# danihae/bio-image-unet

Hardware: AMD Instinct MI355X
Metric: voxels/sec fwd+bwd (higher is better)
Workload: dtype bf16; 1 GPU; cfg4: UNet3D(in_channels=1, out_channels=1, n_filter=32) input (4, 1, 128, 128, 128) per GPU, train step = forward + reference loss + backward + Adam; parallelism=dp1

## Files before the change

### bio_image_unet_amd/csrc/biu_api.hip

```cpp
#include "biu_common.h"
#include "biu_internal.h"

#include <stdlib.h>
#include <string.h>

static const char* const kOffTokens[] = {
    "conv_fwd", "conv_dgrad", "conv_wgrad", "convt_fwd", "convt_dgrad", "convt_wgrad", "convt_all", "c1", "c1_mfma", "cat",
    "fused_stats", "wgrad_bn", "dgrad_bnred", "pool_pair", "pool_pipe", "pool_bnred", "head_bnred", "ksplit", "m16", "m16x2", "rr16",
    "wroll", "wroll16", "wroll2d", "upconv", "foldt", "foldall", "foldck8", "foldgemm", "croll", "froll", "prepack", "wsplitbn",
    "capturefork", "sidechain",
};
constexpr int kNumOffTokens = sizeof(kOffTokens) / sizeof(kOffTokens[0]);
static_assert(kNumOffTokens <= 64, "BiuEnv::off holds one bit per token");

static int off_index(const char* tok, size_t n) {
    for (int i = 0; i < kNumOffTokens; ++i)
        if (strlen(kOffTokens[i]) == n && strncmp(kOffTokens[i], tok, n) == 0) return i;
    return -1;
}
static void env_unknown(const char* var, const char* val, int n) {
    fprintf(stderr, "[biu] %s: unknown %s '%.*s' ignored\n", var, strcmp(var, "BIU_DISABLE") == 0 ? "token" : "value", n, val);
}
static bool parse_int(const char* s, int* v) {
    char* end = nullptr;
    const long r = strtol(s, &end, 10);
    if (end == s || *end) return false;
    *v = (int)r;
    return true;
}

const BiuEnv& biu_env() {
    static const BiuEnv env = [] {
        BiuEnv v{0, false, false, 0, 2, 0, 128};
        if (const char* p = getenv("BIU_DISABLE")) {
            while (true) {
                const size_t n = strcspn(p, ",");
                const int i = off_index(p, n);
                if (i >= 0) v.off |= 1ull << i;
                else if (n > 0) env_unknown("BIU_DISABLE", p, (int)n);
                if (!p[n]) break;
                p += n + 1;
            }
        }
        if (const char* e = getenv("BIU_ROLL"); e && *e) {
            if (strcmp(e, "always") == 0) v.roll_always = true;
            else env_unknown("BIU_ROLL", e, (int)strlen(e));
        }
        if (const char* e = getenv("BIU_FOLDT"); e && *e) {
            int n = 0;
            if (strcmp(e, "always") == 0) v.foldt_always = true;
            else if (strncmp(e, "cmax:", 5) == 0 && parse_int(e + 5, &n) && n > 0) v.foldt_cmax = n;
            else if (strcmp(e, "size") != 0) env_unknown("BIU_FOLDT", e, (int)strlen(e));
        }
        if (const char* e = getenv("BIU_FP32_PRODUCTS"); e && *e) {
            if (strcmp(e, "exact") == 0) v.fp32_products = 0;
            else if (strcmp(e, "bf16x3") == 0) v.fp32_products = 1;
            else if (strcmp(e, "bf16x6") != 0) env_unknown("BIU_FP32_PRODUCTS", e, (int)strlen(e));
        }
        if (const char* e = getenv("BIU_FP32_PRODUCTS_3D"); e && *e) {
            if (strcmp(e, "bf16x3") == 0) v.fp32_products_3d = 1;
            else if (strcmp(e, "bf16x6") == 0) v.fp32_products_3d = 2;
            else if (strcmp(e, "exact") != 0) env_unknown("BIU_FP32_PRODUCTS_3D", e, (int)strlen(e));
// ... 497 lines not shown
```

### bio_image_unet_amd/csrc/biu_conv_mfma.hip

```cpp
#include "biu_internal.h"
#include <type_traits>
#include <cstring>
#include <mutex>
#include <cstdlib>

typedef float floatx16 __attribute__((ext_vector_type(16)));
typedef float floatx4 __attribute__((ext_vector_type(4)));
typedef __bf16 bf16x8 __attribute__((ext_vector_type(8)));

template <typename T> struct Frag;
template <> struct Frag<bf16_t> {
    static constexpr int PE = 8;
    __device__ static __forceinline__ void mma(const uint4& a, const uint4& b, floatx16& c) {
        c = __builtin_amdgcn_mfma_f32_32x32x16_bf16(__builtin_bit_cast(bf16x8, a), __builtin_bit_cast(bf16x8, b), c, 0, 0, 0);
    }
    __device__ static __forceinline__ void unpack(const uint4& v, float* f) {
        const unsigned u[4] = {v.x, v.y, v.z, v.w};
#pragma unroll
        for (int i = 0; i < 4; ++i) {
            f[2 * i] = __uint_as_float(u[i] << 16);
            f[2 * i + 1] = __uint_as_float(u[i] & 0xffff0000u);
        }
    }
    __device__ static __forceinline__ uint4 pack(const float* f) {
// ... 2964 lines not shown
            if (tap < TAPS) {
#pragma unroll
                for (int ni = 0; ni < NI; ++ni)
#pragma unroll
                    for (int e = 0; e < 16; ++e) {
                        const int ii = it * CTA + ni * CT + (e & 3) + 8 * (e >> 2) + 4 * hf;
                        if (ii < a.CA) atomicAdd(wsp + ((size_t)tap * a.CA + ii) * a.CB + jj, acc[t2][ni][e]);
                    }
            }
        }
    }
}

typedef unsigned v4u_t __attribute__((ext_vector_type(4)));
__device__ __forceinline__ void bload_lds16(unsigned voff, v4u_t rsrc, unsigned lds_base_uniform) {
    unsigned keep;
    asm volatile("s_mov_b32 %0, m0\n\ts_mov_b32 m0, %3\n\ts_nop 0\n\tbuffer_load_dwordx4 %1, %2, 0 offen lds\n\ts_mov_b32 m0, %0"
                 : "=&s"(keep)
                 : "v"(voff), "s"(rsrc), "s"(lds_base_uniform)
                 : "memory");
}
__device__ __forceinline__ v4u_t raw_rsrc(const void* base, unsigned bytes) {
    const unsigned long long pa = (unsigned long long)base;
    v4u_t r;
    r[0] = __builtin_amdgcn_readfirstlane((unsigned)pa);
    r[1] = __builtin_amdgcn_readfirstlane((unsigned)(pa >> 32) & 0xffffu);
    r[2] = __builtin_amdgcn_readfirstlane(bytes);
    r[3] = 0x00020000u;
    return r;
}

#ifndef BIU_WROLL_ABL
#define BIU_WROLL_ABL 0
#endif
#ifndef BIU_DIAG_WAVE
#define BIU_DIAG_WAVE 0
#endif
constexpr int WR_TD = 2, WR_TH = 8, WR_TW = 16;
constexpr int WR_HH = WR_TH + 2, WR_HW = WR_TW + 2, WR_PL = WR_HH * WR_HW;
constexpr int WR_RS = 64;
constexpr int WR_PLB = WR_PL * WR_RS;
constexpr int WR_NBI = 24;
constexpr int WR_PAIRB = WR_NBI * 1024;
constexpr int WR_NPAIR = 4;
constexpr int WR_BV = WR_TD * WR_TH * WR_TW;
constexpr int WR_AB = WR_BV * WR_RS;
constexpr int WR_NAI = WR_AB / 1024;
constexpr int WR_NABUF = 3;
constexpr size_t WR_LDS = (size_t)WR_NPAIR * WR_PAIRB + WR_NABUF * WR_AB + 9 * 32 * sizeof(float);

__device__ __forceinline__ unsigned opaque_s(unsigned x) { asm volatile("" : "+s"(x)); return x; }
template <int N> __device__ __forceinline__ void wait_vmcnt() { asm volatile("s_waitcnt vmcnt(%0)" ::"n"(N) : "memory"); }

template <bool BNF, bool K2D, bool A16 = false>
__global__ __launch_bounds__(512, 2) void k_wgrad_roll(WgradArgs a) {
    static_assert(!(K2D && A16), "the 16-channel plain operand form exists for volumes only");
    using T = bf16_t;
    using F = Frag<T>;
    constexpr int TD = WR_TD, TH = WR_TH, TW = WR_TW, HW = WR_HW, PL = WR_PL, RS = WR_RS, PLB = WR_PLB, PAIRB = WR_PAIRB;
    constexpr int CT = 32, PE = 8, TAPS = K2D ? 9 : 27, IPW = K2D ? 3 : 4, NROW = TD * TH;
    constexpr int NBK = WR_NBI / 8, NAK = A16 ? 1 : WR_NAI / 8;
    constexpr int NACC = A16 ? 6 : IPW;

    extern __shared__ __attribute__((aligned(16))) uint4 lds[];
    char* bring = (char*)lds;
    char* abuf = bring + WR_NPAIR * PAIRB;
    float* lxf = (float*)(abuf + WR_NABUF * WR_AB);
    constexpr int LB = 0, LBN = 3 * CT;

    const int tid = threadIdx.x, lane = tid & 63;
    const int wave = __builtin_amdgcn_readfirstlane(tid >> 6);
    const int it = blockIdx.y / a.jt_count, jt = a.jt_begin + blockIdx.y % a.jt_count;
    const int piece = lane & 3;
    const int apc = A16 ? (piece & 1) : piece;
    const int ac0 = it * CT + apc * PE, bc0 = jt * CT + piece * PE;
    const bool apiece_ok = ac0 < a.CA, bpiece_ok = bc0 < a.CB;
    const bool b_src1 = a.pb1 && jt * CT >= a.bsplit;
    const char* pb_ = b_src1 ? a.pb1 : a.pb;
    const int bpitch_ = b_src1 ? a.bpitch1 : a.bpitch;
    const int bc_local = bc0 - (b_src1 ? a.bsplit : 0);
    const float* bs_ = b_src1 ? a.bs1_ : a.bs_;
    const float* bb_ = b_src1 ? a.bb1_ : a.bb_;
    const float* bl_ = b_src1 ? a.bl1_ : a.bl_;
    const bool b_xf = bs_ != nullptr;
    constexpr bool bn_fused = BNF;
    const bool wb = bn_fused && a.write_back;
    if (tid < CT && bn_fused) {
        const int ca = it * CT + tid;
        const bool ok = ca < a.CA;
        lxf[LBN + 0 * CT + tid] = ok ? a.bn_scale[ca] : 1.f;
        lxf[LBN + 1 * CT + tid] = ok ? a.bn_shift[ca] : 0.f;
        lxf[LBN + 2 * CT + tid] = (ok && a.bn_slope) ? a.bn_slope[ca] : 1.f;
        lxf[LBN + 3 * CT + tid] = ok ? a.bn_cA[ca] : 0.f;
        lxf[LBN + 4 * CT + tid] = ok ? a.bn_cB[ca] : 0.f;
        lxf[LBN + 5 * CT + tid] = ok ? a.bn_cC[ca] : 0.f;
    }
    if (tid < CT) {
        const int cb = jt * CT + tid;
        const int cbl = cb - (b_src1 ? a.bsplit : 0);
        lxf[LB + 0 * CT + tid] = (b_xf && cb < a.CB) ? bs_[cbl] : 1.f;
        lxf[LB + 1 * CT + tid] = (b_xf && cb < a.CB) ? bb_[cbl] : 0.f;
        lxf[LB + 2 * CT + tid] = (b_xf && cb < a.CB) ? bl_[cbl] : 1.f;
    }

    floatx16 acc[NACC];
#pragma unroll
    for (int t = 0; t < NACC; ++t)
#pragma unroll
        for (int e = 0; e < 16; ++e) acc[t][e] = 0.f;
    const int wkd = wave / 3, wkw = wave % 3;
    const bool has_x = A16 ? (wave < 4) : (!K2D && wave < 3);
    int tapid[IPW];
#pragma unroll
    for (int t = 0; t < IPW; ++t) {
        if constexpr (K2D) tapid[t] = (wave < 6) ? t * 3 + wkw : TAPS;
        else tapid[t] = (t < 3) ? (wkd * 3 + t) * 3 + wkw : (has_x ? (2 * 3 + wave) * 3 + 2 : TAPS);
    }
    int ab_lane;
    {
        const int g = lane >> 4, li = lane & 15, qrow = li >> 2, p = li & 3, cg = g & 1, h = g >> 1;
        ab_lane = (8 * h + qrow) * RS + (16 * cg + 4 * p) * 2;
    }

    unsigned bco[NBK], aco[NAK];
#pragma unroll
    for (int k = 0; k < NBK; ++k) {
        const int v = ((wave + 8 * k) * 64 + lane) >> 2;
        const int pl = v / PL, r = v % PL;
        bco[k] = (v < 2 * PL && bpiece_ok) ? (unsigned)(pl | ((r / HW) << 10) | ((r % HW) << 20)) : 0xffffffffu;
    }
#pragma unroll
    for (int k = 0; k < NAK; ++k) {
        const int v = ((wave + 8 * k) * 64 + lane) >> 2;
        if constexpr (A16) aco[k] = apiece_ok ? (unsigned)((piece >> 1) | ((v >> 4) << 10) | ((v & 15) << 20)) : 0xffffffffu;
        else aco[k] = apiece_ok ? (unsigned)((v >> 7) | (((v >> 4) & 7) << 10) | ((v & 15) << 20)) : 0xffffffffu;
    }
    const unsigned rowA = (unsigned)a.apitch * 2u, rowY = (unsigned)a.ypitch * 2u, rowB = (unsigned)bpitch_ * 2u;
    const size_t sampA = (size_t)a.GD * a.GH * a.GW * rowA, sampY = (size_t)a.GD * a.GH * a.GW * rowY, sampB = (size_t)a.BD * a.BH * a.BW * rowB;
    const unsigned lds0 = (unsigned)(uintptr_t)((__attribute__((address_space(3))) void*)bring);

    int cn = 0, ch0 = 0, cw0 = 0;
    v4u_t rsB, rsA;
    __amdgpu_buffer_rsrc_t rsAr, rsYr;
    struct Slot { unsigned bmask, amask; uint4 pa[BNF ? NAK : 1], pyv[BNF ? NAK : 1]; };
    Slot sl0, sl1;
    sl0.bmask = sl0.amask = sl1.bmask = sl1.amask = 0;
    unsigned bbase[NBK], abase_[NAK], ybase_[BNF ? NAK : 1];
    unsigned planeB = 0, planeA = 0, planeY = 0;
    auto set_column = [&](int col) __attribute__((always_inline)) {
        int c = col;
        const int wb_ = c % a.nbw; c /= a.nbw;
        const int hb = c % a.nbh;
        cn = c / a.nbh;
        ch0 = hb * TH; cw0 = wb_ * TW;
        rsB = raw_rsrc(pb_ + (size_t)cn * sampB, (unsigned)sampB);
        rsA = raw_rsrc(a.pa + (size_t)cn * sampA, (unsigned)sampA);
        rsAr = __builtin_amdgcn_make_buffer_rsrc((void*)(a.pa + (size_t)cn * sampA), 0, (int)(unsigned)sampA, 0x00020000);
        rsYr = __builtin_amdgcn_make_buffer_rsrc((void*)(a.py + (size_t)cn * sampY), 0, bn_fused ? (int)(unsigned)sampY : 0, 0x00020000);
        planeB = (unsigned)(a.BH * a.BW) * rowB; planeA = (unsigned)(a.GH * a.GW) * rowA; planeY = (unsigned)(a.GH * a.GW) * rowY;
#pragma unroll
        for (int k = 0; k < NBK; ++k) {
            const unsigned x = bco[k];
            const int gh = ch0 - 1 + (int)((x >> 10) & 1023u), gw = cw0 - 1 + (int)(x >> 20);
            const bool ok = x != 0xffffffffu && (unsigned)gh < (unsigned)a.BH && (unsigned)gw < (unsigned)a.BW;
            bbase[k] = ok ? (unsigned)(gh * a.BW + gw) * rowB + (unsigned)bc_local * 2u + (x & 1023u) * planeB : 0xffffffffu;
        }
#pragma unroll
        for (int k = 0; k < NAK; ++k) {
            const unsigned x = aco[k];
            const int gh = ch0 + (int)((x >> 10) & 1023u), gw = cw0 + (int)(x >> 20);
            const bool ok = x != 0xffffffffu && gh < a.GH && gw < a.GW;
            const unsigned vox = (unsigned)(gh * a.GW + gw);
            abase_[k] = ok ? vox * rowA + (unsigned)ac0 * 2u + (x & 1023u) * planeA : 0xffffffffu;
            if constexpr (BNF) ybase_[k] = ok ? vox * rowY + (unsigned)ac0 * 2u + (x & 1023u) * planeY : 0xffffffffu;
        }
    };
    struct FetchCtx { int pair, buf; bool bd0, bd1, ad0, ad1; unsigned dofB, dofA, dofY; };
    auto fetch_ctx = [&](int pair, int gp0, int buf, int d0) __attribute__((always_inline)) -> FetchCtx {
        FetchCtx f;
        f.pair = pair; f.buf = buf;
        f.bd0 = (unsigned)gp0 < (unsigned)a.BD; f.bd1 = (unsigned)(gp0 + 1) < (unsigned)a.BD;
        f.ad0 = d0 < a.GD; f.ad1 = d0 + 1 < a.GD;
        f.dofB = opaque_s((unsigned)gp0 * planeB);
        f.dofA = opaque_s((unsigned)d0 * planeA); f.dofY = opaque_s((unsigned)d0 * planeY);
        f.pair = (int)opaque_s((unsigned)pair); f.buf = (int)opaque_s((unsigned)buf);
        return f;
    };
    auto fetch_piece = [&](Slot& sl, const FetchCtx& f, int i) __attribute__((always_inline)) {
        if (i < NBK) {
            const int k = i;
            const bool ok = bbase[k] != 0xffffffffu && ((bco[k] & 1u) ? f.bd1 : f.bd0);
            bload_lds16(ok ? bbase[k] + f.dofB : 0xffffffffu, rsB, lds0 + (unsigned)(f.pair * PAIRB + (wave + 8 * k) * 1024));
            sl.bmask = (k == 0 ? 0u : sl.bmask) | (ok ? (1u << k) : 0u);
        } else {
            const int k = i - NBK;
            const bool ok = abase_[k] != 0xffffffffu && ((aco[k] & 1u) ? f.ad1 : f.ad0);
            if constexpr (BNF) {
                const auto v0 = __builtin_amdgcn_raw_buffer_load_b128(rsAr, ok ? (int)(abase_[k] + f.dofA) : -1, 0, 0);
                const auto v1 = __builtin_amdgcn_raw_buffer_load_b128(rsYr, ok ? (int)(ybase_[k] + f.dofY) : -1, 0, 0);
                sl.pa[k] = make_uint4(v0[0], v0[1], v0[2], v0[3]);
                sl.pyv[k] = make_uint4(v1[0], v1[1], v1[2], v1[3]);
            } else {
                bload_lds16(ok ? abase_[k] + f.dofA : 0xffffffffu, rsA, lds0 + (unsigned)(WR_NPAIR * PAIRB + f.buf * WR_AB + (wave + 8 * k) * 1024));
            }
            sl.amask = (k == 0 ? 0u : sl.amask) | (ok ? (1u << k) : 0u);
        }
    };
    auto fetch_all = [&](Slot& sl, const FetchCtx& f, bool with_a) __attribute__((always_inline)) {
#pragma unroll
        for (int i = 0; i < NBK + NAK; ++i)
            if (i < NBK || with_a) fetch_piece(sl, f, i);
    };
    auto finish = [&](Slot& sl, int pair_, int buf_, int d0, bool with_a) __attribute__((always_inline)) {
        const int pair = (int)opaque_s((unsigned)pair_), buf = (int)opaque_s((unsigned)buf_);
        const unsigned dofA = opaque_s((unsigned)d0 * planeA);
        if (b_xf) {
            float sc[PE], sh[PE], sl_[PE];
#pragma unroll
            for (int e = 0; e < PE; ++e) { sc[e] = lxf[LB + piece * PE + e]; sh[e] = lxf[LB + CT + piece * PE + e]; sl_[e] = lxf[LB + 2 * CT + piece * PE + e]; }
#pragma unroll
            for (int k = 0; k < NBK; ++k) {
                if ((sl.bmask >> k) & 1u) {
                    uint4* p_ = (uint4*)(bring + pair * PAIRB + (wave + 8 * k) * 1024 + lane * 16);
                    *p_ = apply_xf16<T, PE>(*p_, sc, sh, sl_);
                }
            }
        }
        __builtin_amdgcn_sched_barrier(0);
        if constexpr (BNF) if (with_a) {
            {
                float ks[PE], kh[PE], kl[PE];
#pragma unroll
                for (int e = 0; e < PE; ++e) { ks[e] = lxf[LBN + apc * PE + e]; kh[e] = lxf[LBN + CT + apc * PE + e]; kl[e] = lxf[LBN + 2 * CT + apc * PE + e]; }
#pragma unroll
                for (int k = 0; k < NAK; ++k) {
                    if ((sl.amask >> k) & 1u) {
                        float g[PE], yy[PE];
                        F::unpack(sl.pa[k], g);
                        F::unpack(sl.pyv[k], yy);
#pragma unroll
                        for (int e = 0; e < PE; ++e) g[e] *= (fmaf(ks[e], yy[e], kh[e]) > 0.f ? 1.f : kl[e]);
                        sl.pa[k] = F::pack(g);
                    }
                }
            }
            __builtin_amdgcn_sched_barrier(0);
            {
                float ka[PE], kb[PE], kc[PE];
#pragma unroll
                for (int e = 0; e < PE; ++e) { ka[e] = lxf[LBN + 3 * CT + apc * PE + e]; kb[e] = lxf[LBN + 4 * CT + apc * PE + e]; kc[e] = lxf[LBN + 5 * CT + apc * PE + e]; }
#pragma unroll
                for (int k = 0; k < NAK; ++k) {
                    uint4 v = make_uint4(0, 0, 0, 0);
                    const bool ok = (sl.amask >> k) & 1u;
                    if (ok) {
                        float g[PE], yy[PE];
                        F::unpack(sl.pa[k], g);
                        F::unpack(sl.pyv[k], yy);
#pragma unroll
                        for (int e = 0; e < PE; ++e) g[e] = fmaf(ka[e], g[e], fmaf(kb[e], yy[e], kc[e]));
                        v = F::pack(g);
                    }
                    if (wb) __builtin_amdgcn_raw_buffer_store_b128(v4u_t{v.x, v.y, v.z, v.w}, rsAr, ok ? (int)(abase_[k] + dofA) : -1, 0, 0);
                    *(uint4*)(abuf + buf * WR_AB + (wave + 8 * k) * 1024 + lane * 16) = v;
                }
            }
        }
    };
    auto wait_older = [&](bool younger_in_flight) __attribute__((always_inline)) {
        if (!younger_in_flight) { wait_vmcnt<0>(); return; }
        if (wb) wait_vmcnt<NAK + NBK + 2 * NAK>();
        else if (bn_fused) wait_vmcnt<NBK + 2 * NAK>();
        else wait_vmcnt<NBK + NAK>();
    };

    typedef bf16x4 __attribute__((address_space(3))) * lp;
    auto rd = [&](const char* p_) -> bf16x8 {
        const bf16x4 v0 = __builtin_amdgcn_ds_read_tr16_b64_v4bf16((lp)(p_));
        const bf16x4 v1 = __builtin_amdgcn_ds_read_tr16_b64_v4bf16((lp)(p_ + 4 * RS));
        return __builtin_shufflevector(v0, v1, 0, 1, 2, 3, 4, 5, 6, 7);
    };
    auto mfma_step = [&](auto has_x_c, int s4, int buf, auto&& issue) __attribute__((always_inline)) {
        constexpr bool HAS_X = decltype(has_x_c)::value;
        auto pj = [&](int j) -> const char* { return bring + opaque_s((unsigned)(((s4 + (j >> 1)) & 3) * PAIRB + (j & 1) * PLB)); };
        if constexpr (A16) {
            const int uj = wave & 3, ukw = wave >> 2;
            const char* b0 = pj(uj) + ukw * RS + ab_lane;
            const char* c0 = pj(uj) + 2 * RS + ab_lane;
            const char* ab = abuf + opaque_s((unsigned)(buf * WR_AB)) + ab_lane;
            bf16x8 ring[4], ring2[HAS_X ? 4 : 1], faa[2];
            faa[0] = rd(ab);
#pragma unroll
            for (int j = 0; j < 3; ++j) {
                ring[j] = rd(b0 + j * HW * RS);
                if constexpr (HAS_X) ring2[j] = rd(c0 + j * HW * RS);
            }
#pragma unroll
            for (int r = 0; r < TH; ++r) {
                if (r + 1 < TH) {
                    faa[(r + 1) & 1] = rd(ab + (r + 1) * 16 * RS);
                    ring[(r + 3) & 3] = rd(b0 + (r + 3) * HW * RS);
                    if constexpr (HAS_X) ring2[(r + 3) & 3] = rd(c0 + (r + 3) * HW * RS);
                }
#pragma unroll
                for (int tb = 0; tb < 3; ++tb) acc[tb] = __builtin_amdgcn_mfma_f32_32x32x16_bf16(faa[r & 1], ring[(r + tb) & 3], acc[tb], 0, 0, 0);
                if constexpr (HAS_X) {
#pragma unroll
                    for (int tb = 0; tb < 3; ++tb) acc[3 + tb] = __builtin_amdgcn_mfma_f32_32x32x16_bf16(faa[r & 1], ring2[(r + tb) & 3], acc[3 + tb], 0, 0, 0);
                }
                if ((r & 1) == 0 && r / 2 < NBK + NAK) issue(r / 2);
                __builtin_amdgcn_sched_barrier(0);
            }
            return;
        }
        if constexpr (K2D) {
            if (wave < 6) {
                const char* b0 = pj(wkd + 1) + wkw * RS + ab_lane;
                const char* ab = abuf + opaque_s((unsigned)(buf * WR_AB + wkd * TH * 16 * RS)) + ab_lane;
                bf16x8 ring[4], faa[2];
                faa[0] = rd(ab);
#pragma unroll
                for (int j = 0; j < 3; ++j) ring[j] = rd(b0 + j * HW * RS);
#pragma unroll
                for (int r = 0; r < TH; ++r) {
                    if (r + 1 < TH) {
                        faa[(r + 1) & 1] = rd(ab + (r + 1) * 16 * RS);
                        ring[(r + 3) & 3] = rd(b0 + (r + 3) * HW * RS);
                    }
#pragma unroll
                    for (int tb = 0; tb < 3; ++tb) acc[tb] = __builtin_amdgcn_mfma_f32_32x32x16_bf16(faa[r & 1], ring[(r + tb) & 3], acc[tb], 0, 0, 0);
                    if (r < NBK + NAK) issue(r);
                    __builtin_amdgcn_sched_barrier(0);
                }
            } else {
#pragma unroll
                for (int i = 0; i < NBK + NAK; ++i) issue(i);
            }
// ... 48 lines not shown
    const unsigned long long t0c_ = tprev_, t0r_ = __builtin_amdgcn_s_memrealtime();
#define RSTAMP(k_) do { if (wdiag && (tid & 63) == 0 && (tid >> 6) == (BIU_DIAG_WAVE)) { unsigned long long now_ = __builtin_readcyclecounter(); dsum_[k_] += now_ - tprev_; tprev_ = now_; } } while (0)
#else
#define RSTAMP(k_) do { } while (0)
#endif
    auto step = [&](Slot& mine, Slot& other, int s) __attribute__((always_inline)) {
        const bool f2 = (s + 2 < nsteps) && !((BIU_WROLL_ABL & 1) && s >= 1);
        const bool f1 = (s + 1 < nsteps) && !((BIU_WROLL_ABL & 1) && s >= 2);
        RSTAMP(0);
        const FetchCtx fc = fetch_ctx((s + 3) & 3, 2 * s + 5, (s + 2) % 3, 2 * s + 4);
        RSTAMP(1);
        auto issue = [&](int i) __attribute__((always_inline)) { if (f2) fetch_piece(mine, fc, i); };
        if (has_x) mfma_step(std::true_type{}, s & 3, s % 3, issue); else mfma_step(std::false_type{}, s & 3, s % 3, issue);
        __builtin_amdgcn_sched_barrier(0);
        RSTAMP(2);
        if (f1) {
            wait_older(f2);
            RSTAMP(3);
            finish(other, (s + 2) & 3, (s + 1) % 3, 2 * s + 2, true);
        }
        RSTAMP(4);
        __syncthreads();
        RSTAMP(5);
#ifdef BIU_DIAG
        dsum_[7] += 1;
#endif
    };
    __syncthreads();
    for (int kc = 0;; ++kc) {
        const int col = column_of(kc);
        if (col >= ncols) break;
        set_column(col);
        fetch_all(sl0, fetch_ctx(0, -1, 0, 0), false);
        wait_vmcnt<0>();
        finish(sl0, 0, 0, 0, false);
        fetch_all(sl0, fetch_ctx(1, 1, 0, 0), true);
        if (nsteps > 1) fetch_all(sl1, fetch_ctx(2, 3, 1, 2), true);
        wait_vmcnt<0>();
        finish(sl0, 1, 0, 0, true);
        __syncthreads();
        for (int s = 0; s < nsteps; s += 2) {
            step(sl0, sl1, s);
            if (s + 1 < nsteps) step(sl1, sl0, s + 1);
        }
    }

#ifdef BIU_DIAG
    if (wdiag && (tid & 63) == 0 && (tid >> 6) == (BIU_DIAG_WAVE)) {
        for (int q_ = 0; q_ < 8; ++q_) atomicAdd(wdiag + q_, dsum_[q_]);
        atomicAdd(wdiag + 8, __builtin_readcyclecounter() - t0c_);
        atomicAdd(wdiag + 9, __builtin_amdgcn_s_memrealtime() - t0r_);
    }
#endif
    const int hf = lane >> 5;
    const int jj = jt * CT + (lane & 31);
    if constexpr (A16) {
        const int uj = wave & 3;
        if (jj < a.CB) {
#pragma unroll
            for (int u = 0; u < 2; ++u) {
                if (u == 1 && !has_x) break;
                const int kw = u ? 2 : (wave >> 2);
#pragma unroll
                for (int tb = 0; tb < 3; ++tb)
#pragma unroll
                    for (int e = 0; e < 16; ++e) {
                        const int kd = uj - (e >> 3), ii = (e & 3) + 8 * ((e >> 2) & 1) + 4 * hf;
                        if (kd >= 0 && kd <= 2 && ii < a.CA) atomicAdd(a.ws + ((size_t)((kd * 3 + tb) * 3 + kw) * a.CA + ii) * a.CB + jj, acc[u * 3 + tb][e]);
                    }
            }
        }
        return;
    }
    if (jj < a.CB) {
#pragma unroll
        for (int t2 = 0; t2 < IPW; ++t2) {
            const int tap = tapid[t2];
            if (tap < TAPS) {
#pragma unroll
                for (int e = 0; e < 16; ++e) {
                    const int ii = it * CT + (e & 3) + 8 * (e >> 2) + 4 * hf;
                    if (ii < a.CA) atomicAdd(a.ws + ((size_t)tap * a.CA + ii) * a.CB + jj, acc[t2][e]);
                }
            }
        }
    }
}

static bool wroll_fits(const WgradArgs& a) {
    const int ncols = a.N * ((a.GH + WR_TH - 1) / WR_TH) * ((a.GW + WR_TW - 1) / WR_TW);
    return a.GD >= 8 && ncols >= 8;
}
static bool wroll2d_fits(const WgradArgs& a, i64 bytesA, i64 bytesB, i64 bytesY) {
    const int ncols = ((a.GH + WR_TH - 1) / WR_TH) * ((a.GW + WR_TW - 1) / WR_TW);
    return a.N >= 8 && ncols >= 8 && a.CA * a.CB > 1024 && bytesA < BIU_MAX_SAMPLE_BYTES && bytesB < BIU_MAX_SAMPLE_BYTES && bytesY < BIU_MAX_SAMPLE_BYTES;
}

static int launch_wgrad_roll(WgradArgs a, hipStream_t st, bool k2d = false) {
    if (k2d) { a.GD = a.BD = a.N; a.N = 1; }
    const bool a16 = !k2d && a.CA == 16 && !biu_off("wroll16");
    a.nbd = 1;
    a.nbh = (a.GH + WR_TH - 1) / WR_TH;
    a.nbw = (a.GW + WR_TW - 1) / WR_TW;
    const int ncols = a.N * a.nbh * a.nbw;
    a.nbricks = ncols;
    const int nit = (a.CA + 31) / 32;
    a.njt = (a.CB + 31) / 32;
    a.bricks_per_block = 0;
#ifdef BIU_DIAG
    a.diag = biu_diag_buffer;
#else
    a.diag = nullptr;
#endif
    static bool attr_set = false;
    if (!attr_set) {
        if (hipFuncSetAttribute((const void*)k_wgrad_roll<false, false>, hipFuncAttributeMaxDynamicSharedMemorySize, (int)WR_LDS) != hipSuccess ||
            hipFuncSetAttribute((const void*)k_wgrad_roll<true, false>, hipFuncAttributeMaxDynamicSharedMemorySize, (int)WR_LDS) != hipSuccess ||
            hipFuncSetAttribute((const void*)k_wgrad_roll<false, true>, hipFuncAttributeMaxDynamicSharedMemorySize, (int)WR_LDS) != hipSuccess ||
            hipFuncSetAttribute((const void*)k_wgrad_roll<true, true>, hipFuncAttributeMaxDynamicSharedMemorySize, (int)WR_LDS) != hipSuccess ||
            hipFuncSetAttribute((const void*)k_wgrad_roll<false, false, true>, hipFuncAttributeMaxDynamicSharedMemorySize, (int)WR_LDS) != hipSuccess ||
            hipFuncSetAttribute((const void*)k_wgrad_roll<true, false, true>, hipFuncAttributeMaxDynamicSharedMemorySize, (int)WR_LDS) != hipSuccess)
            return biu_fail(BIU_ERR_LAUNCH, "wgrad_roll: cannot reserve %zu bytes of LDS", WR_LDS);
        attr_set = true;
    }
    auto launch = [&](int jt_begin, int jt_count, int write_back, bool with_bn) {
        WgradArgs b = a;
        if (!with_bn) b.py = nullptr;
        b.jt_begin = jt_begin; b.jt_count = jt_count; b.write_back = write_back;
        const int pairs = nit * jt_count;
        int g = num_cus() / pairs;
        if (g >= 16) g = grid_per_column(num_cus(), pairs);
        if (g < 1) g = 1;
        if (g > ncols) g = ncols;
        if (k2d) {
            if (with_bn) hipLaunchKernelGGL((k_wgrad_roll<true, true>), dim3(g, pairs), dim3(512), WR_LDS, st, b);
            else hipLaunchKernelGGL((k_wgrad_roll<false, true>), dim3(g, pairs), dim3(512), WR_LDS, st, b);
        } else if (a16) {
            if (with_bn) hipLaunchKernelGGL((k_wgrad_roll<true, false, true>), dim3(g, pairs), dim3(512), WR_LDS, st, b);
            else hipLaunchKernelGGL((k_wgrad_roll<false, false, true>), dim3(g, pairs), dim3(512), WR_LDS, st, b);
        } else {
            if (with_bn) hipLaunchKernelGGL((k_wgrad_roll<true, false>), dim3(g, pairs), dim3(512), WR_LDS, st, b);
            else hipLaunchKernelGGL((k_wgrad_roll<false, false>), dim3(g, pairs), dim3(512), WR_LDS, st, b);
        }
    };
    if (a.py && a.njt > 1) {
        launch(0, 1, 1, true);
        BIU_CHECK_LAUNCH("wgrad_roll");
        launch(1, a.njt - 1, 0, false);
    } else {
        launch(0, a.njt, a.py ? 1 : 0, a.py != nullptr);
    }
    BIU_CHECK_LAUNCH("wgrad_roll");
    return BIU_OK;
}

__global__ void k_wgrad_finalize(const float* __restrict__ ws, int rows, int cols, int taps, float* __restrict__ dw, int ld_cols = 0, int c_off = 0) {
    const size_t total = (size_t)rows * cols * taps;
    for (size_t i = (size_t)blockIdx.x * blockDim.x + threadIdx.x; i < total; i += (size_t)gridDim.x * blockDim.x) {
        const int tap = (int)(i % taps);
        const size_t r = i / taps;
        const int c = (int)(r % cols);
        const int rr = (int)(r / cols);
        const size_t o = ld_cols > 0 ? ((size_t)rr * ld_cols + c_off + c) * taps + tap : i;
        dw[o] = ws[((size_t)tap * rows + rr) * cols + c];
    }
}

__global__ void k_zero_f32(float* __restrict__ p, size_t n, float* __restrict__ q, int nq) {
    for (size_t i = (size_t)blockIdx.x * blockDim.x + threadIdx.x; i < n; i += (size_t)gridDim.x * blockDim.x) p[i] = 0.f;
    if (q && blockIdx.x == 0)
        for (int i = threadIdx.x; i < nq; i += blockDim.x) q[i] = 0.f;
}
static int zero_ws(void* ws, size_t bytes, float* extra, int nextra, hipStream_t st) {
    const size_t n = bytes / sizeof(float);
    hipLaunchKernelGGL(k_zero_f32, dim3(grid_for((i64)n, 256, 1024)), dim3(256), 0, st, (float*)ws, n, extra, nextra);
    if (hipGetLastError() != hipSuccess) return biu_fail(BIU_ERR_LAUNCH, "wgrad: zero-fill launch failed");
    return BIU_OK;
}

static bool wgrad_chan_ok(int cin, int cout) { return cin >= 16 && cin % 8 == 0 && cout >= 16 && cout % 8 == 0; }

static size_t wgrad_acc_bytes(int cin, int cout, int taps) { return (((size_t)cin * cout * taps * sizeof(float)) + 255) & ~(size_t)255; }

size_t biu_mfma_wgrad_workspace(int cin, int cout, int kd, int kh, int kw, int dtype) {
    if (!wgrad_chan_ok(cin, cout)) return 0;
    const size_t red = biu_chan_sum_workspace(cout);
    if (kh == 3 && kw == 3 && (kd == 1 || kd == 3)) return wgrad_acc_bytes(cin, cout, kd * 9) + red;
    if (kh == 2 && kw == 2 && (kd == 1 || kd == 2)) return wgrad_acc_bytes(cin, cout, kd * 4) + red;
    return 0;
// ... 65 lines not shown
        launch(0, a.njt, a.py ? 1 : 0, a.py != nullptr);
    }
    BIU_CHECK_LAUNCH("wgrad_pipe");
    return BIU_OK;
}

static int wgrad_xf(const biu_xform* xf, const float** s, const float** b, const float** l) {
    const bool has = xf && (xf->scale || xf->shift || xf->slope);
    if (has) BIU_REQUIRE(xf->scale && xf->shift && xf->slope, BIU_ERR_UNSUPPORTED, "wgrad_mfma: partial biu_xform");
    *s = has ? xf->scale : nullptr;
    *b = has ? xf->shift : nullptr;
    *l = has ? xf->slope : nullptr;
    return BIU_OK;
}

int biu_mfma_wgrad(const biu_act* x, const biu_xform* xf, const biu_act* dy, int kd, int kh, int kw, float* dw, float* dbias,
                   void* ws, size_t ws_bytes, int dtype, hipStream_t st, const BnBwdFuse* bn, const biu_act* x1, const biu_xform* xf1,
                   int dw_ld_cols, int dw_c_off) {
    WgradArgs a;
    int rc_ = BIU_OK;
    if (bn && !biu_off("wsplitbn") && dtype == BIU_BF16 && kd == 3 && x->c + (x1 ? x1->c : 0) > 32 && nvox(dy) <= 4 * 32 * 32 * 32) {
        rc_ = biu_bn_bwd_apply(dy, bn->y, bn->scale, bn->shift, bn->slope, bn->cA, bn->cB, bn->cC, dy, dtype, (biu_stream)st);
        if (rc_ != BIU_OK) return rc_;
        bn = nullptr;
    }
    if (bn) {
        a.py = (const char*)bn->y->p; a.ypitch = bn->y->pitch;
        a.bn_scale = bn->scale; a.bn_shift = bn->shift; a.bn_slope = bn->slope;
        a.bn_cA = bn->cA; a.bn_cB = bn->cB; a.bn_cC = bn->cC;
    } else {
        a.py = nullptr; a.ypitch = 0;
        a.bn_scale = a.bn_shift = a.bn_slope = a.bn_cA = a.bn_cB = a.bn_cC = nullptr;
    }
    a.pa = (const char*)dy->p;  a.apitch = dy->pitch;  a.CA = dy->c;
    a.pb = (const char*)x->p;   a.bpitch = x->pitch;   a.CB = x->c;
    a.dbias_out = nullptr;
    a.fold_par = -1;
    a.pb1 = nullptr; a.bpitch1 = 0; a.bsplit = 0; a.bs1_ = a.bb1_ = a.bl1_ = nullptr;
    if (x1) {
        a.pb1 = (const char*)x1->p; a.bpitch1 = x1->pitch; a.bsplit = x->c; a.CB = x->c + x1->c;
        rc_ = wgrad_xf(xf1, &a.bs1_, &a.bb1_, &a.bl1_);
        if (rc_) return rc_;
    }
    a.ws = (float*)ws;
    a.as_ = a.ab_ = a.al_ = nullptr;
    int rc = wgrad_xf(xf, &a.bs_, &a.bb_, &a.bl_);
    if (rc) return rc;
    a.N = x->n;
    a.GD = a.BD = x->d; a.GH = a.BH = x->h; a.GW = a.BW = x->w;
    const int taps = kd * 9;
    const size_t need = wgrad_acc_bytes(a.CA, a.CB, taps);
    BIU_REQUIRE(ws_bytes >= need + (dbias ? biu_chan_sum_workspace(dy->c) : 0), BIU_ERR_WORKSPACE, "wgrad_mfma: workspace %zu too small", ws_bytes);
    if (int zr = zero_ws(ws, need, nullptr, 0, st)) return zr;
    if (dtype == BIU_BF16 && kd == 3 && a.CB == 16 && !x1 && !biu_off("rr16")) rc = launch_wgrad<bf16_t, 3, 3, 1, 4, 8, 16, 1, 1, true>(a, st);
    else if (dtype == BIU_BF16 && kd == 3 && !biu_off("wroll") && wroll_fits(a)) rc = launch_wgrad_roll(a, st);
    else if (dtype == BIU_BF16 && kd == 1 && !biu_off("wroll") && !biu_off("wroll2d") &&
             wroll2d_fits(a, (i64)nvox(dy) * dy->pitch * 2, (i64)nvox(x) * x->pitch * 2 > (x1 ? (i64)nvox(x1) * x1->pitch * 2 : 0) ? (i64)nvox(x) * x->pitch * 2 : (i64)nvox(x1) * x1->pitch * 2,
                          bn ? (i64)nvox(bn->y) * bn->y->pitch * 2 : 0))
        rc = launch_wgrad_roll(a, st, true);
    else if (dtype == BIU_BF16) rc = (kd == 3) ? launch_wgrad<bf16_t, 3, 3, 1, 4, 8, 16, 1>(a, st) : launch_wgrad<bf16_t, 1, 3, 1, 1, 16, 32, 4>(a, st);
    else if (kd == 1 && x3_mode_of(kd, dtype) == 2) rc = launch_wgrad<f32x6_t, 1, 3, 1, 1, 16, 16, 4>(a, st);
    else if (kd == 1 && x3_mode_of(kd, dtype) == 1) rc = launch_wgrad<f32x3_t, 1, 3, 1, 1, 16, 16, 4>(a, st);
    else if (kd == 3 && x3_mode_of(kd, dtype) == 2) rc = launch_wgrad<f32x6_t, 3, 3, 1, 2, 4, 16, 1>(a, st);
    else if (kd == 3 && x3_mode_of(kd, dtype) == 1) rc = launch_wgrad<f32x3_t, 3, 3, 1, 2, 4, 16, 1>(a, st);
    else rc = (kd == 3) ? launch_wgrad<float, 3, 3, 1, 4, 4, 16, 1>(a, st) : launch_wgrad<float, 1, 3, 1, 1, 16, 16, 4>(a, st);
    if (rc != BIU_OK) return rc;
    hipLaunchKernelGGL(k_wgrad_finalize, dim3(grid_for((i64)a.CA * a.CB * taps, 256, 2048)), dim3(256), 0, st, (const float*)ws,
                       a.CA, a.CB, taps, dw, dw_ld_cols, dw_c_off);
    BIU_CHECK_LAUNCH("wgrad_finalize");
    if (dbias) return biu_chan_sum_vec(dy, dbias, (char*)ws + need, dtype, st);
    return BIU_OK;
}

__global__ void k_upconv_wgrad_unfold(const float* __restrict__ ws, size_t slice_f, int cout, int cin, float* __restrict__ dw) {
    const size_t total = (size_t)cout * cin * 27;
    for (size_t idx = (size_t)blockIdx.x * blockDim.x + threadIdx.x; idx < total; idx += (size_t)gridDim.x * blockDim.x) {
        const int k = (int)(idx % 27);
        const size_t r = idx / 27;
        const int ci = (int)(r % cin), co = (int)(r / cin);
        const int kk[3] = {k / 9, (k / 3) % 3, k % 3};
        float sum = 0.f;
        for (int p = 0; p < 8; ++p) {
            int t = 0;
#pragma unroll
            for (int ax = 0; ax < 3; ++ax) {
                const int pa = (p >> (2 - ax)) & 1;
                const int ta = pa == 0 ? (kk[ax] >= 1 ? 1 : 0) : (kk[ax] == 2 ? 1 : 0);
                t |= ta << (2 - ax);
            }
            sum += ws[(size_t)p * slice_f + ((size_t)t * cout + co) * cin + ci];
        }
        dw[idx] = sum;
    }
}
size_t biu_mfma_upconv_wgrad_workspace(int cin, int cout, int dtype) {
    if ((dtype != BIU_BF16 && dtype != BIU_F32) || !wgrad_chan_ok(cin, cout)) return 0;
    return 8 * wgrad_acc_bytes(cout, cin, 8);
}
int biu_mfma_upconv_wgrad(const biu_act* x, const biu_xform* xf, const biu_act* dy, float* dw, void* ws, size_t ws_bytes, int dtype,
                          hipStream_t st, const BnBwdFuse* bn) {
    WgradArgs a;
    if (bn) {
        a.py = (const char*)bn->y->p; a.ypitch = bn->y->pitch;
        a.bn_scale = bn->scale; a.bn_shift = bn->shift; a.bn_slope = bn->slope;
        a.bn_cA = bn->cA; a.bn_cB = bn->cB; a.bn_cC = bn->cC;
    } else {
        a.py = nullptr; a.ypitch = 0;
// ... 294 lines not shown
```

Baseline: 733.9 million voxels/s.

## Add 16x16x32 MFMA variant of rolled wgrad kernel for 16-channel convolutions

Adds an F16 template mode to the rolled 3D weight-gradient kernel that uses 16x16x32 bf16 MFMA with transposed LDS reads, remapping the operand fetch pieces so 16-channel A or B operands don't waste half of a 32x32 tile. The dispatcher now sends kd=3 bf16 wgrad with CA==16 or CB==16 to this path ahead of the existing rr16 and a16 paths, with a new 'wgrad16' disable token. It aims to cut wasted MFMA work and padding on the first and last UNet levels (n_filter=32 gives 16-channel layers). In exchange it adds more atomics per output and a more complex load and fetch mapping, which risks correctness or register pressure.

```diff
diff --git a/bio_image_unet_amd/csrc/biu_api.hip b/bio_image_unet_amd/csrc/biu_api.hip
--- a/bio_image_unet_amd/csrc/biu_api.hip
+++ b/bio_image_unet_amd/csrc/biu_api.hip
@@ -7,7 +7,7 @@
 static const char* const kOffTokens[] = {
     "conv_fwd", "conv_dgrad", "conv_wgrad", "convt_fwd", "convt_dgrad", "convt_wgrad", "convt_all", "c1", "c1_mfma", "cat",
     "fused_stats", "wgrad_bn", "dgrad_bnred", "pool_pair", "pool_pipe", "pool_bnred", "head_bnred", "ksplit", "m16", "m16x2", "rr16",
-    "wroll", "wroll16", "wroll2d", "upconv", "foldt", "foldall", "foldck8", "foldgemm", "croll", "froll", "prepack", "wsplitbn",
+    "wroll", "wroll16", "wroll2d", "wgrad16", "upconv", "foldt", "foldall", "foldck8", "foldgemm", "croll", "froll", "prepack", "wsplitbn",
     "capturefork", "sidechain",
 };
 constexpr int kNumOffTokens = sizeof(kOffTokens) / sizeof(kOffTokens[0]);
diff --git a/bio_image_unet_amd/csrc/biu_conv_mfma.hip b/bio_image_unet_amd/csrc/biu_conv_mfma.hip
--- a/bio_image_unet_amd/csrc/biu_conv_mfma.hip
+++ b/bio_image_unet_amd/csrc/biu_conv_mfma.hip
@@ -3040,15 +3040,17 @@
 __device__ __forceinline__ unsigned opaque_s(unsigned x) { asm volatile("" : "+s"(x)); return x; }
 template <int N> __device__ __forceinline__ void wait_vmcnt() { asm volatile("s_waitcnt vmcnt(%0)" ::"n"(N) : "memory"); }
 
-template <bool BNF, bool K2D, bool A16 = false>
+template <bool BNF, bool K2D, bool A16 = false, int F16 = 0>
 __global__ __launch_bounds__(512, 2) void k_wgrad_roll(WgradArgs a) {
     static_assert(!(K2D && A16), "the 16-channel plain operand form exists for volumes only");
+    static_assert(F16 == 0 || (!K2D && !A16), "the 16x16x32 form exists for volumes only");
     using T = bf16_t;
     using F = Frag<T>;
     constexpr int TD = WR_TD, TH = WR_TH, TW = WR_TW, HW = WR_HW, PL = WR_PL, RS = WR_RS, PLB = WR_PLB, PAIRB = WR_PAIRB;
     constexpr int CT = 32, PE = 8, TAPS = K2D ? 9 : 27, IPW = K2D ? 3 : 4, NROW = TD * TH;
-    constexpr int NBK = WR_NBI / 8, NAK = A16 ? 1 : WR_NAI / 8;
-    constexpr int NACC = A16 ? 6 : IPW;
+    constexpr int NBK = WR_NBI / 8, NAK = (A16 || F16 == 1) ? 1 : WR_NAI / 8;
+    constexpr int NACC = F16 ? 1 : A16 ? 6 : IPW;
+    constexpr int NHA = F16 == 2 ? 2 : 1, NHB = F16 == 1 ? 2 : 1;
 
     extern __shared__ __attribute__((aligned(16))) uint4 lds[];
     char* bring = (char*)lds;
@@ -3060,7 +3062,7 @@
     const int wave = __builtin_amdgcn_readfirstlane(tid >> 6);
     const int it = blockIdx.y / a.jt_count, jt = a.jt_begin + blockIdx.y % a.jt_count;
     const int piece = lane & 3;
-    const int apc = A16 ? (piece & 1) : piece;
+    const int apc = F16 ? (lane & 1) : A16 ? (piece & 1) : piece;
     const int ac0 = it * CT + apc * PE, bc0 = jt * CT + piece * PE;
     const bool apiece_ok = ac0 < a.CA, bpiece_ok = bc0 < a.CB;
     const bool b_src1 = a.pb1 && jt * CT >= a.bsplit;
@@ -3096,6 +3098,11 @@
     for (int t = 0; t < NACC; ++t)
 #pragma unroll
         for (int e = 0; e < 16; ++e) acc[t][e] = 0.f;
+    floatx4 acc4[F16 ? 4 * NHA * NHB : 1];
+#pragma unroll
+    for (int t = 0; t < (F16 ? 4 * NHA * NHB : 1); ++t)
+#pragma unroll
+        for (int e = 0; e < 4; ++e) acc4[t][e] = 0.f;
     const int wkd = wave / 3, wkw = wave % 3;
     const bool has_x = A16 ? (wave < 4) : (!K2D && wave < 3);
     int tapid[IPW];
@@ -3110,15 +3117,28 @@
         ab_lane = (8 * h + qrow) * RS + (16 * cg + 4 * p) * 2;
     }
 
+    auto f16_bpiece = [&](int k) -> int { return 2 * ((wave + 8 * k) / 12) + (lane & 1); };
+    auto f16_apiece = [&](int k) -> int { return 2 * k + (lane & 1); };
     unsigned bco[NBK], aco[NAK];
 #pragma unroll
     for (int k = 0; k < NBK; ++k) {
+        if constexpr (F16 != 0) {
+            const int v = ((wave + 8 * k) % 12) * 32 + (lane >> 1);
+            const int pl = v / PL, r = v % PL;
+            bco[k] = (v < 2 * PL && jt * CT + f16_bpiece(k) * PE < a.CB) ? (unsigned)(pl | ((r / HW) << 10) | ((r % HW) << 20)) : 0xffffffffu;
+            continue;
+        }
         const int v = ((wave + 8 * k) * 64 + lane) >> 2;
         const int pl = v / PL, r = v % PL;
         bco[k] = (v < 2 * PL && bpiece_ok) ? (unsigned)(pl | ((r / HW) << 10) | ((r % HW) << 20)) : 0xffffffffu;
     }
 #pragma unroll
     for (int k = 0; k < NAK; ++k) {
+        if constexpr (F16 != 0) {
+            const int v = wave * 32 + (lane >> 1);
+            aco[k] = (it * CT + f16_apiece(k) * PE < a.CA) ? (unsigned)((v >> 7) | (((v >> 4) & 7) << 10) | ((v & 15) << 20)) : 0xffffffffu;
+            continue;
+        }
         const int v = ((wave + 8 * k) * 64 + lane) >> 2;
         if constexpr (A16) aco[k] = apiece_ok ? (unsigned)((piece >> 1) | ((v >> 4) << 10) | ((v & 15) << 20)) : 0xffffffffu;
         else aco[k] = apiece_ok ? (unsigned)((v >> 7) | (((v >> 4) & 7) << 10) | ((v & 15) << 20)) : 0xffffffffu;
@@ -3151,7 +3171,8 @@
             const unsigned x = bco[k];
             const int gh = ch0 - 1 + (int)((x >> 10) & 1023u), gw = cw0 - 1 + (int)(x >> 20);
             const bool ok = x != 0xffffffffu && (unsigned)gh < (unsigned)a.BH && (unsigned)gw < (unsigned)a.BW;
-            bbase[k] = ok ? (unsigned)(gh * a.BW + gw) * rowB + (unsigned)bc_local * 2u + (x & 1023u) * planeB : 0xffffffffu;
+            const int bcl = F16 ? jt * CT + f16_bpiece(k) * PE - (b_src1 ? a.bsplit : 0) : bc_local;
+            bbase[k] = ok ? (unsigned)(gh * a.BW + gw) * rowB + (unsigned)bcl * 2u + (x & 1023u) * planeB : 0xffffffffu;
         }
 #pragma unroll
         for (int k = 0; k < NAK; ++k) {
@@ -3159,8 +3180,9 @@
             const int gh = ch0 + (int)((x >> 10) & 1023u), gw = cw0 + (int)(x >> 20);
             const bool ok = x != 0xffffffffu && gh < a.GH && gw < a.GW;
             const unsigned vox = (unsigned)(gh * a.GW + gw);
-            abase_[k] = ok ? vox * rowA + (unsigned)ac0 * 2u + (x & 1023u) * planeA : 0xffffffffu;
-            if constexpr (BNF) ybase_[k] = ok ? vox * rowY + (unsigned)ac0 * 2u + (x & 1023u) * planeY : 0xffffffffu;
+            const int acc0 = F16 ? it * CT + f16_apiece(k) * PE : ac0;
+            abase_[k] = ok ? vox * rowA + (unsigned)acc0 * 2u + (x & 1023u) * planeA : 0xffffffffu;
+            if constexpr (BNF) ybase_[k] = ok ? vox * rowY + (unsigned)acc0 * 2u + (x & 1023u) * planeY : 0xffffffffu;
         }
     };
     struct FetchCtx { int pair, buf; bool bd0, bd1, ad0, ad1; unsigned dofB, dofA, dofY; };
@@ -3202,7 +3224,19 @@
     auto finish = [&](Slot& sl, int pair_, int buf_, int d0, bool with_a) __attribute__((always_inline)) {
         const int pair = (int)opaque_s((unsigned)pair_), buf = (int)opaque_s((unsigned)buf_);
         const unsigned dofA = opaque_s((unsigned)d0 * planeA);
-        if (b_xf) {
+        if (F16 != 0 && b_xf) {
+#pragma unroll
+            for (int k = 0; k < NBK; ++k) {
+                if ((sl.bmask >> k) & 1u) {
+                    const int pc = f16_bpiece(k);
+                    float sc[PE], sh[PE], sl_[PE];
+#pragma unroll
+                    for (int e = 0; e < PE; ++e) { sc[e] = lxf[LB + pc * PE + e]; sh[e] = lxf[LB + CT + pc * PE + e]; sl_[e] = lxf[LB + 2 * CT + pc * PE + e]; }
+                    uint4* p_ = (uint4*)(bring + pair * PAIRB + (wave + 8 * k) * 1024 + lane * 16);
+                    *p_ = apply_xf16<T, PE>(*p_, sc, sh, sl_);
+                }
+            }
+        } else if (b_xf) {
             float sc[PE], sh[PE], sl_[PE];
 #pragma unroll
             for (int e = 0; e < PE; ++e) { sc[e] = lxf[LB + piece * PE + e]; sh[e] = lxf[LB + CT + piece * PE + e]; sl_[e] = lxf[LB + 2 * CT + piece * PE + e]; }
@@ -3222,6 +3256,10 @@
                 for (int e = 0; e < PE; ++e) { ks[e] = lxf[LBN + apc * PE + e]; kh[e] = lxf[LBN + CT + apc * PE + e]; kl[e] = lxf[LBN + 2 * CT + apc * PE + e]; }
 #pragma unroll
                 for (int k = 0; k < NAK; ++k) {
+                    if (F16 != 0 && k > 0) {
+#pragma unroll
+                        for (int e = 0; e < PE; ++e) { const int pc = f16_apiece(k); ks[e] = lxf[LBN + pc * PE + e]; kh[e] = lxf[LBN + CT + pc * PE + e]; kl[e] = lxf[LBN + 2 * CT + pc * PE + e]; }
+                    }
                     if ((sl.amask >> k) & 1u) {
                         float g[PE], yy[PE];
                         F::unpack(sl.pa[k], g);
@@ -3239,6 +3277,10 @@
                 for (int e = 0; e < PE; ++e) { ka[e] = lxf[LBN + 3 * CT + apc * PE + e]; kb[e] = lxf[LBN + 4 * CT + apc * PE + e]; kc[e] = lxf[LBN + 5 * CT + apc * PE + e]; }
 #pragma unroll
                 for (int k = 0; k < NAK; ++k) {
+                    if (F16 != 0 && k > 0) {
+#pragma unroll
+                        for (int e = 0; e < PE; ++e) { const int pc = f16_apiece(k); ka[e] = lxf[LBN + 3 * CT + pc * PE + e]; kb[e] = lxf[LBN + 4 * CT + pc * PE + e]; kc[e] = lxf[LBN + 5 * CT + pc * PE + e]; }
+                    }
                     uint4 v = make_uint4(0, 0, 0, 0);
                     const bool ok = (sl.amask >> k) & 1u;
                     if (ok) {
@@ -3271,6 +3313,63 @@
     auto mfma_step = [&](auto has_x_c, int s4, int buf, auto&& issue) __attribute__((always_inline)) {
         constexpr bool HAS_X = decltype(has_x_c)::value;
         auto pj = [&](int j) -> const char* { return bring + opaque_s((unsigned)(((s4 + (j >> 1)) & 3) * PAIRB + (j & 1) * PLB)); };
+        if constexpr (F16 != 0) {
+            const int P = lane >> 5;
+            const unsigned lofs = (unsigned)((4 * ((lane >> 4) & 1) + ((lane >> 2) & 3)) * 32 + 8 * (lane & 3));
+            auto plj = [&](int j) -> unsigned { return (unsigned)(((s4 + (j >> 1)) & 3) * PAIRB + (j & 1) * (PL * 32)); };
+            const char* b0 = bring + plj(wkd + P) + (unsigned)(wkw * 32) + lofs;
+            const char* x0 = bring + plj(2 + P) + (unsigned)((wave * HW + 2) * 32) + lofs;
+            const char* ab = abuf + opaque_s((unsigned)(buf * WR_AB)) + (unsigned)(P * 128 * 32) + lofs;
+            auto rd16 = [&](const char* p_) -> bf16x8 {
+                const bf16x4 v0 = __builtin_amdgcn_ds_read_tr16_b64_v4bf16((lp)(p_));
+                const bf16x4 v1 = __builtin_amdgcn_ds_read_tr16_b64_v4bf16((lp)(p_ + 8 * 32));
+                return __builtin_shufflevector(v0, v1, 0, 1, 2, 3, 4, 5, 6, 7);
+            };
+            constexpr int HB = 12 * 1024, HA = WR_BV * 32, RB = HW * 32, RA = TW * 32;
+            bf16x8 fa[2][NHA], ring[4][NHB], fx[HAS_X ? 2 : 1][NHB];
+#pragma unroll
+            for (int h = 0; h < NHA; ++h) fa[0][h] = rd16(ab + h * HA);
+#pragma unroll
+            for (int j = 0; j < 3; ++j)
+#pragma unroll
+                for (int h = 0; h < NHB; ++h) ring[j][h] = rd16(b0 + j * RB + h * HB);
+            if constexpr (HAS_X) {
+#pragma unroll
+                for (int h = 0; h < NHB; ++h) fx[0][h] = rd16(x0 + h * HB);
+            }
+#pragma unroll
+            for (int r = 0; r < TH; ++r) {
+                if (r + 1 < TH) {
+#pragma unroll
+                    for (int h = 0; h < NHA; ++h) fa[(r + 1) & 1][h] = rd16(ab + (r + 1) * RA + h * HA);
+#pragma unroll
+                    for (int h = 0; h < NHB; ++h) ring[(r + 3) & 3][h] = rd16(b0 + (r + 3) * RB + h * HB);
+                    if constexpr (HAS_X) {
+#pragma unroll
+                        for (int h = 0; h < NHB; ++h) fx[(r + 1) & 1][h] = rd16(x0 + (r + 1) * RB + h * HB);
+                    }
+                }
+#pragma unroll
+                for (int tb = 0; tb < 3; ++tb)
+#pragma unroll
+                    for (int ha = 0; ha < NHA; ++ha)
+#pragma unroll
+                        for (int hb = 0; hb < NHB; ++hb)
+                            acc4[(tb * NHA + ha) * NHB + hb] = __builtin_amdgcn_mfma_f32_16x16x32_bf16(fa[r & 1][ha], ring[(r + tb) & 3][hb], acc4[(tb * NHA + ha) * NHB + hb], 0, 0, 0);
+                if constexpr (HAS_X) {
+#pragma unroll
+                    for (int ha = 0; ha < NHA; ++ha)
+#pragma unroll
+                        for (int hb = 0; hb < NHB; ++hb)
+                            acc4[(3 * NHA + ha) * NHB + hb] = __builtin_amdgcn_mfma_f32_16x16x32_bf16(fa[r & 1][ha], fx[r & 1][hb], acc4[(3 * NHA + ha) * NHB + hb], 0, 0, 0);
+                }
+#pragma unroll
+                for (int i = 0; i < NBK + NAK; ++i)
+                    if (i * TH / (NBK + NAK) == r) issue(i);
+                __builtin_amdgcn_sched_barrier(0);
+            }
+            return;
+        }
         if constexpr (A16) {
             const int uj = wave & 3, ukw = wave >> 2;
             const char* b0 = pj(uj) + ukw * RS + ab_lane;
@@ -3425,6 +3524,25 @@
         atomicAdd(wdiag + 9, __builtin_amdgcn_s_memrealtime() - t0r_);
     }
 #endif
+    if constexpr (F16 != 0) {
+#pragma unroll
+        for (int t = 0; t < 4; ++t) {
+            const int tap = t < 3 ? (wkd * 3 + t) * 3 + wkw : (has_x ? (2 * 3 + wave) * 3 + 2 : TAPS);
+            if (tap >= TAPS) continue;
+#pragma unroll
+            for (int ha = 0; ha < NHA; ++ha)
+#pragma unroll
+                for (int hb = 0; hb < NHB; ++hb) {
+                    const int j = jt * CT + 16 * hb + (lane & 15);
+#pragma unroll
+                    for (int e = 0; e < 4; ++e) {
+                        const int i = it * CT + 16 * ha + 4 * (lane >> 4) + e;
+                        if (i < a.CA && j < a.CB) atomicAdd(a.ws + ((size_t)tap * a.CA + i) * a.CB + j, acc4[(t * NHA + ha) * NHB + hb][e]);
+                    }
+                }
+        }
+        return;
+    }
     const int hf = lane >> 5;
     const int jj = jt * CT + (lane & 31);
     if constexpr (A16) {
@@ -3469,9 +3587,9 @@
     return a.N >= 8 && ncols >= 8 && a.CA * a.CB > 1024 && bytesA < BIU_MAX_SAMPLE_BYTES && bytesB < BIU_MAX_SAMPLE_BYTES && bytesY < BIU_MAX_SAMPLE_BYTES;
 }
 
-static int launch_wgrad_roll(WgradArgs a, hipStream_t st, bool k2d = false) {
+static int launch_wgrad_roll(WgradArgs a, hipStream_t st, bool k2d = false, int f16 = 0) {
     if (k2d) { a.GD = a.BD = a.N; a.N = 1; }
-    const bool a16 = !k2d && a.CA == 16 && !biu_off("wroll16");
+    const bool a16 = !k2d && !f16 && a.CA == 16 && !biu_off("wroll16");
     a.nbd = 1;
     a.nbh = (a.GH + WR_TH - 1) / WR_TH;
     a.nbw = (a.GW + WR_TW - 1) / WR_TW;
@@ -3492,7 +3610,11 @@
             hipFuncSetAttribute((const void*)k_wgrad_roll<false, true>, hipFuncAttributeMaxDynamicSharedMemorySize, (int)WR_LDS) != hipSuccess ||
             hipFuncSetAttribute((const void*)k_wgrad_roll<true, true>, hipFuncAttributeMaxDynamicSharedMemorySize, (int)WR_LDS) != hipSuccess ||
             hipFuncSetAttribute((const void*)k_wgrad_roll<false, false, true>, hipFuncAttributeMaxDynamicSharedMemorySize, (int)WR_LDS) != hipSuccess ||
-            hipFuncSetAttribute((const void*)k_wgrad_roll<true, false, true>, hipFuncAttributeMaxDynamicSharedMemorySize, (int)WR_LDS) != hipSuccess)
+            hipFuncSetAttribute((const void*)k_wgrad_roll<true, false, true>, hipFuncAttributeMaxDynamicSharedMemorySize, (int)WR_LDS) != hipSuccess ||
+            hipFuncSetAttribute((const void*)k_wgrad_roll<false, false, false, 1>, hipFuncAttributeMaxDynamicSharedMemorySize, (int)WR_LDS) != hipSuccess ||
+            hipFuncSetAttribute((const void*)k_wgrad_roll<true, false, false, 1>, hipFuncAttributeMaxDynamicSharedMemorySize, (int)WR_LDS) != hipSuccess ||
+            hipFuncSetAttribute((const void*)k_wgrad_roll<false, false, false, 2>, hipFuncAttributeMaxDynamicSharedMemorySize, (int)WR_LDS) != hipSuccess ||
+            hipFuncSetAttribute((const void*)k_wgrad_roll<true, false, false, 2>, hipFuncAttributeMaxDynamicSharedMemorySize, (int)WR_LDS) != hipSuccess)
             return biu_fail(BIU_ERR_LAUNCH, "wgrad_roll: cannot reserve %zu bytes of LDS", WR_LDS);
         attr_set = true;
     }
@@ -3508,6 +3630,12 @@
         if (k2d) {
             if (with_bn) hipLaunchKernelGGL((k_wgrad_roll<true, true>), dim3(g, pairs), dim3(512), WR_LDS, st, b);
             else hipLaunchKernelGGL((k_wgrad_roll<false, true>), dim3(g, pairs), dim3(512), WR_LDS, st, b);
+        } else if (f16 == 1) {
+            if (with_bn) hipLaunchKernelGGL((k_wgrad_roll<true, false, false, 1>), dim3(g, pairs), dim3(512), WR_LDS, st, b);
+            else hipLaunchKernelGGL((k_wgrad_roll<false, false, false, 1>), dim3(g, pairs), dim3(512), WR_LDS, st, b);
+        } else if (f16 == 2) {
+            if (with_bn) hipLaunchKernelGGL((k_wgrad_roll<true, false, false, 2>), dim3(g, pairs), dim3(512), WR_LDS, st, b);
+            else hipLaunchKernelGGL((k_wgrad_roll<false, false, false, 2>), dim3(g, pairs), dim3(512), WR_LDS, st, b);
         } else if (a16) {
             if (with_bn) hipLaunchKernelGGL((k_wgrad_roll<true, false, true>), dim3(g, pairs), dim3(512), WR_LDS, st, b);
             else hipLaunchKernelGGL((k_wgrad_roll<false, false, true>), dim3(g, pairs), dim3(512), WR_LDS, st, b);
@@ -3679,7 +3807,9 @@
     const size_t need = wgrad_acc_bytes(a.CA, a.CB, taps);
     BIU_REQUIRE(ws_bytes >= need + (dbias ? biu_chan_sum_workspace(dy->c) : 0), BIU_ERR_WORKSPACE, "wgrad_mfma: workspace %zu too small", ws_bytes);
     if (int zr = zero_ws(ws, need, nullptr, 0, st)) return zr;
-    if (dtype == BIU_BF16 && kd == 3 && a.CB == 16 && !x1 && !biu_off("rr16")) rc = launch_wgrad<bf16_t, 3, 3, 1, 4, 8, 16, 1, 1, true>(a, st);
+    if (dtype == BIU_BF16 && kd == 3 && (a.CA == 16 || (a.CB == 16 && !x1)) && !biu_off("wgrad16") && !biu_off("wroll") && wroll_fits(a))
+        rc = launch_wgrad_roll(a, st, false, a.CA == 16 ? 1 : 2);
+    else if (dtype == BIU_BF16 && kd == 3 && a.CB == 16 && !x1 && !biu_off("rr16")) rc = launch_wgrad<bf16_t, 3, 3, 1, 4, 8, 16, 1, 1, true>(a, st);
     else if (dtype == BIU_BF16 && kd == 3 && !biu_off("wroll") && wroll_fits(a)) rc = launch_wgrad_roll(a, st);
     else if (dtype == BIU_BF16 && kd == 1 && !biu_off("wroll") && !biu_off("wroll2d") &&
              wroll2d_fits(a, (i64)nvox(dy) * dy->pitch * 2, (i64)nvox(x) * x->pitch * 2 > (x1 ? (i64)nvox(x1) * x1->pitch * 2 : 0) ? (i64)nvox(x) * x->pitch * 2 : (i64)nvox(x1) * x1->pitch * 2,
```

Result: no change. 740.0 million voxels/s, median of 6 (+0.8%).
